# xkuubix/MonteCarlo-Gated-MIL

Measured on AMD Instinct MI355X. Metric: bags/sec × MCDO-samples (T=100) at N=2048,d=512; 1/2/4/8-GPU + %HBM roofline, higher is better.
Workload: dtype bf16

## Files before the change

montecarlo-gated-mil_amd/csrc/mcgmil_kernels.h:

```cpp
#pragma once
#include "mcgmil_device.h"

namespace mcgmil {

struct GateParams {
    const void* H;
    long long ldh;
    const int32_t* bag_off;
    int B, T, L, D, C, G, P;
    long long total_samples;
    const void* Wp;
    uint32_t wp_bytes;
    const float* bv;
    const float* bu;
    const float* wa;
    const float* ba;
    float sf, sa;
    uint32_t thr_f, thr_a;
    uint32_t thrx_f;
    uint32_t k0, k1;
    uint32_t bag_base;
    int t_base;
    const uint32_t* bag_ids;
    const int32_t* tile_bag;
// ... 3 lines not shown
    float* logits;
    float* zz;
    float* Y;
    float* A;
    const int32_t* region_off;
    int region_t;
    unsigned long long* stamps;
    unsigned long long* clock;
    long long tile_row0;
};

constexpr int kClockSlots = 1024;
__device__ __forceinline__ void clock_probe(const GateParams& p, int i) {
    if (p.clock && threadIdx.x == 0 && blockIdx.x < (unsigned)kClockSlots) {
        const unsigned long long t = __builtin_amdgcn_s_memtime();
        const unsigned long long r = __builtin_amdgcn_s_memrealtime();
        p.clock[(size_t)blockIdx.x * 4 + 2 * i] = t;
        p.clock[(size_t)blockIdx.x * 4 + 2 * i + 1] = r;
    }
}

#ifdef MCGMIL_STAMPS
#define MCGMIL_STAMP(p, i)                                                                 \
    do {                                                                                    \
        __builtin_amdgcn_sched_barrier(0);                                                  \
        if (threadIdx.x == 0 && (p).stamps)                                                 \
            (p).stamps[(size_t)blockIdx.x * 8 + (i)] = __builtin_amdgcn_s_memtime();        \
        __builtin_amdgcn_sched_barrier(0);                                                  \
    } while (0)
#else
#define MCGMIL_STAMP(p, i) do {} while (0)
#endif


constexpr int kGateThreads = 512;
constexpr int kGateWaves = kGateThreads / kWave;
constexpr int kRowInfo = 6;


template <int BM, int RV = BM>
__device__ __forceinline__ void fill_row_table(const GateParams& p, long long R0, int* rinfo) {
    const int tid = threadIdx.x;
    if (tid >= BM) return;
    const long long R = tid < RV ? R0 + tid : p.total_samples;
    int hrow = -1, t = 0, n = 0, bag = 0, Nb = 0;
    const bool narrow = p.total_samples <= 0xFFFFFFFFll;
    if (R < p.total_samples && p.uniform_rows > 0) {
        const long long per_bag = (long long)p.T * p.uniform_rows;
        Nb = p.uniform_rows;
        if (narrow) {
            const uint32_t r = (uint32_t)R, pb = (uint32_t)per_bag;
            bag = (int)(r / pb);
            const uint32_t local = r - (uint32_t)bag * pb;
            t = (int)(local / (uint32_t)Nb);
            n = (int)(local - (uint32_t)t * (uint32_t)Nb);
        } else {
            bag = (int)(R / per_bag);
            const long long local = R - (long long)bag * per_bag;
            t = (int)(local / Nb);
            n = (int)(local - (long long)t * Nb);
        }
        hrow = bag * Nb + n;
    } else if (R < p.total_samples) {
        if (p.tile_bag) {
            bag = p.tile_bag[R0 / BM];
            while ((long long)p.T * p.bag_off[bag + 1] <= R) ++bag;
        } else {
            bag = find_bag(p.bag_off, p.B, p.T, R);
        }
        const int ob = p.bag_off[bag];
        Nb = p.bag_off[bag + 1] - ob;
        const long long local = R - (long long)p.T * ob;
        if (narrow) {
            t = (int)((uint32_t)local / (uint32_t)Nb);
            n = (int)((uint32_t)local - (uint32_t)t * (uint32_t)Nb);
        } else {
            t = (int)(local / Nb);
            n = (int)(local - (long long)t * Nb);
        }
        hrow = ob + n;
    }
    int* ri = rinfo + kRowInfo * tid;
    ri[0] = hrow; ri[1] = t; ri[2] = n; ri[3] = bag; ri[4] = Nb;
    ri[5] = (int)(p.bag_ids ? p.bag_ids[bag] : p.bag_base + (uint32_t)bag);
}

#ifndef MCGMIL_KERNELS_TEMPLATES_ONLY
__global__ void plan_tiles_kernel(const int32_t* bag_off, int B, int T, long long total_samples,
                                  int BM, long long tiles, int32_t* tile_bag) {
    const long long i = (long long)blockIdx.x * blockDim.x + threadIdx.x;
    if (i >= tiles) return;
    const long long R = i * BM;
    tile_bag[i] = R < total_samples ? find_bag(bag_off, B, T, R) : 0;
}
#endif

__device__ __forceinline__ float gated_product_scaled(float ax, float by) {
    ax = fminf(fmaxf(ax, -43.280851226668903f), 43.280851226668903f);
    const float a = __builtin_amdgcn_exp2f(ax);
    const float b = __builtin_amdgcn_exp2f(by);
    const float ia = 1.0f + a;
    return (1.0f - a) * __builtin_amdgcn_rcpf(fmaf(ia, b, ia));
}

#ifndef MCGMIL_DIAG
#define MCGMIL_DIAG 0
#endif
#ifndef MCGMIL_PHILOX_ROUNDS
#define MCGMIL_PHILOX_ROUNDS 10
#endif

constexpr float kM2Log2e = -2.8853900817779268f;
constexpr float kMLog2e = -1.4426950408889634f;

struct HeadVec { f32x4 bv, bu, wa; };

template <int PPW>
__device__ __forceinline__ void load_head_vectors(const GateParams& p, int q0, int lane,
                                                  HeadVec (&hv)[PPW]) {
    const int DB = p.D >> 4;
#pragma unroll
    for (int jp = 0; jp < PPW; ++jp) {
        const int q = q0 + jp < p.P ? q0 + jp : p.P - 1;
        const int g = q / DB, db = q - g * DB;
        const int d0 = db * 16 + 4 * (lane >> 4);
        hv[jp].bv = *reinterpret_cast<const f32x4*>(p.bv + (size_t)g * p.D + d0) * kM2Log2e;
        hv[jp].bu = *reinterpret_cast<const f32x4*>(p.bu + (size_t)g * p.D + d0) * kMLog2e;
        hv[jp].wa = *reinterpret_cast<const f32x4*>(p.wa + (size_t)g * p.D + d0);
    }
}

struct Region {
    int bag, t0, t1, Nb, ob;
    int ntiles;
    long long S, rows;
};

constexpr int kFusedTiles = 32;
constexpr int kFusedHv = 256;
struct alignas(16) FusedConst {
    Region rg;
    uint32_t bagctr;
    int pad0;
    float ba[4];
    int cls[8];
    int pad1[8];
    int4 tile[kFusedTiles];
    float hv[3][kFusedHv];
};

#ifndef MCGMIL_FUSED_HV_LDS
#define MCGMIL_FUSED_HV_LDS 1
#endif
template <int PPW>
__device__ __forceinline__ void load_head_vectors_lds(const FusedConst* fc, int P, int q0, int lane,
                                                      HeadVec (&hv)[PPW]) {
#pragma unroll
    for (int jp = 0; jp < PPW; ++jp) {
        const int q = q0 + jp < P ? q0 + jp : P - 1;
        const int d = 16 * q + 4 * (lane >> 4);
        hv[jp].bv = *reinterpret_cast<const f32x4*>(fc->hv[0] + d);
        hv[jp].bu = *reinterpret_cast<const f32x4*>(fc->hv[1] + d);
        hv[jp].wa = *reinterpret_cast<const f32x4*>(fc->hv[2] + d);
    }
}

template <int RT, int PPW, int MAXC, bool ONE_CLASS, int RTV = RT>
__device__ __forceinline__ void fold_pairs(const GateParams& p, const f32x4 (&acc)[RT][2 * PPW],
                                           int q0, int lane, float (&part)[MAXC][RT],
                                           const HeadVec* pre = nullptr) {
    const int DB = p.D >> 4;
    const float av_s = p.sf * kM2Log2e, au_s = p.sf * kMLog2e;
#pragma unroll
    for (int jp = 0; jp < PPW; ++jp) {
        const int q = q0 + jp;
        if (q >= p.P) break;
        const int col = 16 * q + 4 * (lane >> 4);
        const int g = ONE_CLASS ? 0 : q / DB;
        const int d0 = col - g * p.D;
        f32x4 bvv, buv;
        f32x4 coef[MAXC];
        if (ONE_CLASS && pre) {
            bvv = pre[jp].bv;
            buv = pre[jp].bu;
            coef[0] = pre[jp].wa;
#pragma unroll
            for (int c = 1; c < MAXC; ++c) coef[c] = f32x4{0.f, 0.f, 0.f, 0.f};
        } else {
            bvv = *reinterpret_cast<const f32x4*>(p.bv + col);
            buv = *reinterpret_cast<const f32x4*>(p.bu + col);
            bvv *= kM2Log2e;
            buv *= kMLog2e;
#pragma unroll
            for (int c = 0; c < MAXC; ++c) {
                const int cc = ONE_CLASS ? g : c;
                const bool use = ONE_CLASS ? (c == 0) : ((c < p.C) && (p.G == 1 || c == g));
                const f32x4 w = *reinterpret_cast<const f32x4*>(p.wa + (size_t)(use ? cc : 0) * p.D + d0);
                coef[c] = use ? w : f32x4{0.f, 0.f, 0.f, 0.f};
            }
        }
#pragma unroll
        for (int rt = 0; rt < RTV; ++rt) {
#pragma unroll
            for (int v = 0; v < 4; ++v) {
                const float ax = fmaf(acc[rt][2 * jp][v], av_s, bvv[v]);
                const float by = fmaf(acc[rt][2 * jp + 1][v], au_s, buv[v]);
                if constexpr (ONE_CLASS) {
#if MCGMIL_DIAG & 8
                    part[0][rt] = fmaf(fmaf(ax, coef[0][v], by), ax, part[0][rt]);
                    continue;
#endif
                    const float a = __builtin_amdgcn_exp2f(fminf(fmaxf(ax, -43.280851226668903f),
                                                                 43.280851226668903f));
                    const float b = __builtin_amdgcn_exp2f(by);
                    const float ia = 1.0f + a;
                    const float r = __builtin_amdgcn_rcpf(fmaf(ia, b, ia));
                    part[0][rt] = fmaf(fmaf(-a, coef[0][v], coef[0][v]), r, part[0][rt]);
                } else {
                    const float pr = gated_product_scaled(ax, by);
#pragma unroll
                    for (int c = 0; c < MAXC; ++c) part[c][rt] = fmaf(pr, coef[c][v], part[c][rt]);
                }
            }
        }
    }
}

template <int BM, int MAXC>
__host__ __device__ constexpr int red_floats() { return kGateWaves * MAXC * 4 * BM; }

template <int BM, int MAXC, int ROWS = 16, bool AFFINE = false>
__device__ __forceinline__ void finish_scores(const GateParams& p, long long R0,
                                              float (&part)[MAXC][BM / ROWS], f32x4 zacc,
                                              bool zwave, float* red, float* zred,
                                              const int* rinfo, int one_class, int waves_per_gate,
                                              bool have_keep, bool keep, float* lg_out,
                                              float* z_out, long long obase,
                                              const FusedConst* fc = nullptr, int tile = 0) {
    constexpr int RT = BM / ROWS;
    constexpr int NG = 64 / ROWS;
    const int tid = threadIdx.x, lane = tid & 63, wave = tid >> 6;
    const int ncls = one_class < 0 ? MAXC : 1;
#pragma unroll
    for (int c = 0; c < MAXC; ++c) {
        if (c >= ncls) break;
        const int cls = one_class < 0 ? c : one_class;
        if (cls >= MAXC) break;
        float* dst = red + ((size_t)(wave * MAXC + cls) * NG + lane / ROWS) * BM + (lane % ROWS);
#pragma unroll
        for (int q = 0; q < RT; ++q) dst[ROWS * q] = part[c][q];
    }
    if (zwave && lane < 16) {
#pragma unroll
        for (int c = 0; c < MAXC; ++c) zred[c * BM + wave * 16 + lane] = zacc[c];
    }
    MCGMIL_STAMP(p, 5);
    __syncthreads();
    MCGMIL_STAMP(p, 6);
    const int r = wave * 16 + (lane & 15), c = lane >> 4;
    if (r >= BM || c >= p.C) return;
    int t, n, bag, Nb;
    uint32_t bagc;
    size_t orow;
    float bias;
    if constexpr (AFFINE) {
        const int4 tl = fc->tile[tile];
        t = tl.x, n = tl.y + r, bag = fc->rg.bag, Nb = fc->rg.Nb;
        bagc = fc->bagctr;
        orow = (size_t)(tl.z + r);
        bias = fc->ba[c];
    } else {
        const int* ri = rinfo + kRowInfo * r;
        if (ri[0] < 0) return;
        t = ri[1], n = ri[2], bag = ri[3], Nb = ri[4];
        bagc = (uint32_t)ri[5];
        orow = (size_t)(R0 + r - obase);
        bias = p.ba[c];
    }
    float s = 0.f;
    const int nw = waves_per_gate ? waves_per_gate : kGateWaves;
    for (int k = 0; k < nw; ++k) {
        const int w = waves_per_gate ? c * waves_per_gate + k : k;
        const float* src = red + (size_t)(w * MAXC + c) * NG * BM + r;
#pragma unroll
        for (int g = 0; g < NG; ++g) s += src[g * BM];
    }
    s += bias;
    if (p.keep_att) {
        const size_t abase = (size_t)p.T * p.C * (size_t)p.bag_off[bag];
        keep = p.keep_att[abase + ((size_t)t * p.C + c) * Nb + n] != 0;
    } else if (!have_keep) {
        keep = attention_keep(p.k0, p.k1, bagc, (uint32_t)(p.t_base + t), (uint32_t)c,
                              (uint32_t)n, p.thr_a);
    }
    const size_t o = orow * p.C + c;
    lg_out[o] = s * (keep ? p.sa : 0.f);
    z_out[o] = zred[c * BM + r] * p.sf;
}

constexpr int kSoftmaxRows = 16;

#ifndef MCGMIL_NT_A
#define MCGMIL_NT_A 1
#endif
__device__ __forceinline__ void store_a(float* dst, float v) {
#if MCGMIL_NT_A
    __builtin_nontemporal_store(v, dst);
#else
    *dst = v;
#endif
}

__device__ __forceinline__ void softmax_group(int ltid, bool active, int Nb, int C, const float* lg,
                                              const float* zz, float* Ao, float* Yo, float* sred) {
    const int tid = ltid, lane = ltid & 63, wave = ltid >> 6;
    if (Nb == 0) {
        if (active && tid < C) Yo[tid] = 0.f;
        return;
    }
    const int Nl = active ? Nb : 0;
    if (C == 2 && Nb <= 256 * kSoftmaxRows) {
        float (*sred2)[4] = reinterpret_cast<float (*)[4]>(sred);
        float e0[kSoftmaxRows], e1[kSoftmaxRows];
        float2 zr[kSoftmaxRows];
        float m0 = -INFINITY, m1 = -INFINITY;
#pragma unroll
        for (int k = 0; k < kSoftmaxRows; ++k) {
            const int n = tid + 256 * k;
            float2 l = make_float2(-INFINITY, -INFINITY);
            zr[k] = make_float2(0.f, 0.f);
            if (n < Nl) {
                l = *reinterpret_cast<const float2*>(lg + (size_t)n * 2);
                zr[k] = *reinterpret_cast<const float2*>(zz + (size_t)n * 2);
            }
            e0[k] = l.x;
            e1[k] = l.y;
            m0 = fmaxf(m0, e0[k]);
            m1 = fmaxf(m1, e1[k]);
        }
        m0 = wave_max(m0);
        m1 = wave_max(m1);
        if (lane == 0) { sred2[0][wave] = m0; sred2[1][wave] = m1; }
        __syncthreads();
        m0 = fmaxf(fmaxf(sred2[0][0], sred2[0][1]), fmaxf(sred2[0][2], sred2[0][3]));
        m1 = fmaxf(fmaxf(sred2[1][0], sred2[1][1]), fmaxf(sred2[1][2], sred2[1][3]));
        __syncthreads();
        float s0 = 0.f, y0 = 0.f, s1 = 0.f, y1 = 0.f;
#pragma unroll
        for (int k = 0; k < kSoftmaxRows; ++k) {
            const int n = tid + 256 * k;
            if (n < Nl) {
                const float2 z = zr[k];
                e0[k] = expf(e0[k] - m0);
                e1[k] = expf(e1[k] - m1);
                s0 += e0[k];
                s1 += e1[k];
                y0 = fmaf(e0[k], z.x, y0);
                y1 = fmaf(e1[k], z.y, y1);
            }
        }
        s0 = wave_sum(s0);
        y0 = wave_sum(y0);
        s1 = wave_sum(s1);
        y1 = wave_sum(y1);
        if (lane == 0) {
            sred2[0][wave] = s0; sred2[1][wave] = y0; sred2[2][wave] = s1; sred2[3][wave] = y1;
        }
        __syncthreads();
        s0 = (sred2[0][0] + sred2[0][1]) + (sred2[0][2] + sred2[0][3]);
        y0 = (sred2[1][0] + sred2[1][1]) + (sred2[1][2] + sred2[1][3]);
        s1 = (sred2[2][0] + sred2[2][1]) + (sred2[2][2] + sred2[2][3]);
        y1 = (sred2[3][0] + sred2[3][1]) + (sred2[3][2] + sred2[3][3]);
        __syncthreads();
        const float inv0 = 1.0f / s0, inv1 = 1.0f / s1;
        if (Ao) {
            float* Ao1 = Ao + Nb;
#pragma unroll
            for (int k = 0; k < kSoftmaxRows; ++k) {
                const int n = tid + 256 * k;
                if (n < Nl) {
                    store_a(Ao + n, e0[k] * inv0);
                    store_a(Ao1 + n, e1[k] * inv1);
                }
            }
        }
        if (active && tid == 0) { Yo[0] = y0 * inv0; Yo[1] = y1 * inv1; }
        return;
    }
    float (*sr)[4] = reinterpret_cast<float (*)[4]>(sred);
    for (int c = 0; c < C; ++c) {
        if (Nb <= 256 * kSoftmaxRows) {
            float e[kSoftmaxRows];
            float m = -INFINITY;
#pragma unroll
            for (int k = 0; k < kSoftmaxRows; ++k) {
                const int n = tid + 256 * k;
                e[k] = n < Nl ? lg[(size_t)n * C + c] : -INFINITY;
                m = fmaxf(m, e[k]);
            }
            m = wave_max(m);
            if (lane == 0) sr[0][wave] = m;
            __syncthreads();
            m = fmaxf(fmaxf(sr[0][0], sr[0][1]), fmaxf(sr[0][2], sr[0][3]));
            __syncthreads();
            float s = 0.f, y = 0.f;
#pragma unroll
            for (int k = 0; k < kSoftmaxRows; ++k) {
                const int n = tid + 256 * k;
                if (n < Nl) {
                    e[k] = expf(e[k] - m);
                    s += e[k];
                    y = fmaf(e[k], zz[(size_t)n * C + c], y);
                }
            }
            s = wave_sum(s);
            y = wave_sum(y);
            if (lane == 0) { sr[0][wave] = s; sr[1][wave] = y; }
            __syncthreads();
            s = (sr[0][0] + sr[0][1]) + (sr[0][2] + sr[0][3]);
            y = (sr[1][0] + sr[1][1]) + (sr[1][2] + sr[1][3]);
            __syncthreads();
            const float inv = 1.0f / s;
            if (Ao) {
                float* Aoc = Ao + (size_t)c * Nb;
#pragma unroll
                for (int k = 0; k < kSoftmaxRows; ++k) {
                    const int n = tid + 256 * k;
                    if (n < Nl) store_a(Aoc + n, e[k] * inv);
                }
            }
            if (active && tid == 0) Yo[c] = y * inv;
            continue;
        }
        float m = -INFINITY;
        for (int n = tid; n < Nl; n += 256) m = fmaxf(m, lg[(size_t)n * C + c]);
        m = wave_max(m);
        if (lane == 0) sr[0][wave] = m;
        __syncthreads();
        m = fmaxf(fmaxf(sr[0][0], sr[0][1]), fmaxf(sr[0][2], sr[0][3]));
        __syncthreads();
        float s = 0.f, y = 0.f;
        for (int n = tid; n < Nl; n += 256) {
            const size_t o = (size_t)n * C + c;
            const float e = expf(lg[o] - m);
            s += e;
            y = fmaf(e, zz[o], y);
        }
        s = wave_sum(s);
        y = wave_sum(y);
        if (lane == 0) { sr[0][wave] = s; sr[1][wave] = y; }
        __syncthreads();
        s = (sr[0][0] + sr[0][1]) + (sr[0][2] + sr[0][3]);
        y = (sr[1][0] + sr[1][1]) + (sr[1][2] + sr[1][3]);
        __syncthreads();
        const float inv = 1.0f / s;
        if (Ao) {
            float* Aoc = Ao + (size_t)c * Nb;
            for (int n = tid; n < Nl; n += 256) store_a(Aoc + n, expf(lg[(size_t)n * C + c] - m) * inv);
        }
        if (active && tid == 0) Yo[c] = y * inv;
    }
}

#ifndef MCGMIL_KERNELS_TEMPLATES_ONLY
__global__ __launch_bounds__(256) void softmax_pool_kernel(const int32_t* bag_off, int T, int C,
                                                           const float* logits, const float* zz,
                                                           float* Y, float* A) {
    __shared__ float sred[16];
    const int t = blockIdx.x, b = blockIdx.y;
    const int ob = bag_off[b];
    const int Nb = bag_off[b + 1] - ob;
    const size_t R0 = (size_t)T * ob + (size_t)t * Nb;
    softmax_group(threadIdx.x, true, Nb, C, logits + R0 * C, zz + R0 * C,
                  A ? A + (size_t)T * C * ob + (size_t)t * C * Nb : nullptr,
                  Y + ((size_t)b * T + t) * C, sred);
}
#endif

template <typename E> struct Raw;
template <> struct Raw<__bf16> { uint4 v; };
template <> struct Raw<float> { f32x4 lo, hi; };
__device__ __forceinline__ Raw<__bf16> load_raw(const __bf16* p) {
    Raw<__bf16> r; r.v = *reinterpret_cast<const uint4*>(p); return r;
}
__device__ __forceinline__ Raw<float> load_raw(const float* p) {
    Raw<float> r;
    r.lo = *reinterpret_cast<const f32x4*>(p);
    r.hi = *reinterpret_cast<const f32x4*>(p + 4);
    return r;
}
__device__ __forceinline__ void store_masked(const Raw<__bf16>& h, uint32_t kb, __bf16* dst) {
    uint4 v = h.v;
    v.x &= ((kb & 1u) ? 0x0000FFFFu : 0u) | ((kb & 2u) ? 0xFFFF0000u : 0u);
    v.y &= ((kb & 4u) ? 0x0000FFFFu : 0u) | ((kb & 8u) ? 0xFFFF0000u : 0u);
    v.z &= ((kb & 16u) ? 0x0000FFFFu : 0u) | ((kb & 32u) ? 0xFFFF0000u : 0u);
    v.w &= ((kb & 64u) ? 0x0000FFFFu : 0u) | ((kb & 128u) ? 0xFFFF0000u : 0u);
    *reinterpret_cast<uint4*>(dst) = v;
}
__device__ __forceinline__ void store_masked(const Raw<float>& h, uint32_t kb, float* dst) {
    f32x4 a = h.lo, b = h.hi;
    a.x = (kb & 1u) ? a.x : 0.f;   a.y = (kb & 2u) ? a.y : 0.f;
    a.z = (kb & 4u) ? a.z : 0.f;   a.w = (kb & 8u) ? a.w : 0.f;
    b.x = (kb & 16u) ? b.x : 0.f;  b.y = (kb & 32u) ? b.y : 0.f;
    b.z = (kb & 64u) ? b.z : 0.f;  b.w = (kb & 128u) ? b.w : 0.f;
    *reinterpret_cast<f32x4*>(dst) = a;
    *reinterpret_cast<f32x4*>(dst + 4) = b;
}

__device__ __forceinline__ void store_dropped(const Raw<__bf16>& h, uint4 o, uint32_t thrx,
                                              uint32_t inval, __bf16* dst) {
    uint4 v = h.v;
    v.x = __builtin_amdgcn_bitop3_b32(v.x, drop_mask16x2_flipped(o.x, thrx), inval, 0x10);
    v.y = __builtin_amdgcn_bitop3_b32(v.y, drop_mask16x2(o.y, thrx), inval, 0x10);
    v.z = __builtin_amdgcn_bitop3_b32(v.z, drop_mask16x2_flipped(o.z, thrx), inval, 0x10);
    v.w = __builtin_amdgcn_bitop3_b32(v.w, drop_mask16x2(o.w, thrx), inval, 0x10);
    *reinterpret_cast<uint4*>(dst) = v;
}
__device__ __forceinline__ uint32_t keep_lo(uint32_t m) { return ~(uint32_t)((int32_t)(m << 16) >> 16); }
__device__ __forceinline__ uint32_t keep_hi(uint32_t m) { return ~(uint32_t)((int32_t)m >> 16); }
__device__ __forceinline__ void store_dropped(const Raw<float>& h, uint4 o, uint32_t thrx,
                                              uint32_t inval, float* dst) {
    const uint32_t m0 = drop_mask16x2_flipped(o.x, thrx) | inval, m1 = drop_mask16x2(o.y, thrx) | inval;
    const uint32_t m2 = drop_mask16x2_flipped(o.z, thrx) | inval, m3 = drop_mask16x2(o.w, thrx) | inval;
    f32x4 a = h.lo, b = h.hi;
    a.x = __uint_as_float(__float_as_uint(a.x) & keep_lo(m0));
    a.y = __uint_as_float(__float_as_uint(a.y) & keep_hi(m0));
    a.z = __uint_as_float(__float_as_uint(a.z) & keep_lo(m1));
    a.w = __uint_as_float(__float_as_uint(a.w) & keep_hi(m1));
    b.x = __uint_as_float(__float_as_uint(b.x) & keep_lo(m2));
    b.y = __uint_as_float(__float_as_uint(b.y) & keep_hi(m2));
    b.z = __uint_as_float(__float_as_uint(b.z) & keep_lo(m3));
    b.w = __uint_as_float(__float_as_uint(b.w) & keep_hi(m3));
    *reinterpret_cast<f32x4*>(dst) = a;
    *reinterpret_cast<f32x4*>(dst + 4) = b;
}

constexpr int kPipeBM = 128;
#ifndef MCGMIL_VPM
#define MCGMIL_VPM 2
#endif
constexpr int VPM = MCGMIL_VPM;
#ifndef MCGMIL_SCHED
#define MCGMIL_SCHED 0
#endif
constexpr int HD = 2;
template <typename E>
__host__ __device__ constexpr int pipe_slots() { return 2; }

template <typename E, int MAXC>
__host__ __device__ constexpr size_t pipe_lds_bytes() {
    return (size_t)pipe_slots<E>() * kPipeBM * 32 * sizeof(E) + (size_t)red_floats<kPipeBM, MAXC>() * 4 +
           (size_t)MAXC * kPipeBM * 4 + (size_t)kRowInfo * kPipeBM * 4;
}

template <typename E>
__device__ __forceinline__ void load_classifier_lds(__amdgpu_buffer_rsrc_t wrs, uint32_t zsoff, int KS, E* zw) {
    for (int i = threadIdx.x; i < KS * 64; i += kGateThreads)
        *reinterpret_cast<f32x4*>(zw + (size_t)i * 8) = __builtin_bit_cast(
            f32x4, __builtin_amdgcn_raw_buffer_load_b128(wrs, (uint32_t)i * 8u * (uint32_t)sizeof(E), zsoff, 0));
}

template <typename E, int PPW, int MAXC, bool REPLAY, bool ONE_CLASS, bool EARLY_HV = true,
          bool ZL = false, bool ZLOAD = true, int RTV = kPipeBM / 16, bool AFFINE = false>
__device__ __forceinline__ void pipe_tile(const GateParams& p, long long R0, E* Xs, float* red,
                                          float* zred, const int* rinfo, float* lg_out,
                                          float* z_out, long long obase, E* zw = nullptr,
                                          const FusedConst* fc = nullptr, int tile = 0) {
    constexpr int BM = kPipeBM;
    constexpr int RT = BM / 16;
    constexpr int NJ = 2 * PPW;
    constexpr int SLOT = RT * 64 * 8;
    const int tid = threadIdx.x, lane = tid & 63, wave = tid >> 6;
    const int KS = p.L >> 5;

    int hrow;
    uint32_t cn, ct, cb;
    if constexpr (AFFINE) {
        static_assert(!REPLAY, "the affine rows have no replay masks");
        const int4 tl = fc->tile[tile];
        cn = (uint32_t)(tl.y + wave * 16 + (lane & 15));
        hrow = fc->rg.ob + (int)cn;
        ct = (uint32_t)(p.t_base + tl.x);
        cb = fc->bagctr;
    } else {
        const int* ri = rinfo + kRowInfo * (wave * 16 + (lane & 15));
        hrow = ri[0];
        cn = (uint32_t)ri[2], ct = (uint32_t)(p.t_base + ri[1]), cb = (uint32_t)ri[5];
    }
    const bool valid = AFFINE || hrow >= 0;
    const int kq = lane >> 4;
    const E* hsrc = reinterpret_cast<const E*>(p.H) + (size_t)(valid ? hrow : 0) * p.ldh + kq * 8;
    const uint8_t* kfe = REPLAY ? p.keep_feat + (size_t)(valid ? R0 + wave * 16 + (lane & 15) : 0) *
                                                    (p.L >> 3) + kq
                                : nullptr;

    const uint32_t inval = valid ? 0u : 0xFFFFFFFFu;
    auto stage = [&](int s, const Raw<E>& h, E* slot) {
        if constexpr (REPLAY) {
            const uint32_t kb = kfe[(size_t)(s < KS ? s : KS - 1) * 4];
            store_masked(h, kb & ~inval, slot + tid * 8);
        } else {
#if MCGMIL_DIAG & 4
            const uint4 o = make_uint4(cn * 0x9E3779B9u + (uint32_t)s, ct ^ cb, cn + ct, (uint32_t)s * 77u);
#else
            const uint4 o = philox4x32_10<true, MCGMIL_PHILOX_ROUNDS>((uint32_t)(s * 4 + kq), cn, ct, cb, p.k0, p.k1);
#endif
            store_dropped(h, o, p.thrx_f, inval, slot + tid * 8);
        }
    };

    const __amdgpu_buffer_rsrc_t wrs = make_rsrc(p.Wp, p.wp_bytes);
    const uint32_t tile_bytes = (uint32_t)KS * 512u * (uint32_t)sizeof(E);
    constexpr uint32_t kStepBytes = 512u * (uint32_t)sizeof(E);
    const int q0 = __builtin_amdgcn_readfirstlane(wave) * PPW;
    uint32_t wsoff[NJ];
#pragma unroll
    for (int j = 0; j < NJ; ++j) {
        int q = q0 + (j >> 1);
        q = q < p.P ? q : p.P - 1;
        wsoff[j] = (uint32_t)(2 * q + (j & 1)) * tile_bytes;
    }
    const uint32_t zsoff = (uint32_t)(2 * p.P) * tile_bytes;
    const uint32_t lane_b = (uint32_t)lane * 8u * (uint32_t)sizeof(E);
    auto wfrag = [&](uint32_t soff) { return load_frag_buf<E>(wrs, lane_b, soff); };

    f32x4 acc[RT][NJ];
#pragma unroll
    for (int rt = 0; rt < RT; ++rt)
#pragma unroll
        for (int j = 0; j < NJ; ++j) acc[rt][j] = f32x4{0.f, 0.f, 0.f, 0.f};
    f32x4 zacc = {0.f, 0.f, 0.f, 0.f};

    auto kstep = [&](int s, const E* cur, E* nxt, const Frag<E> (&w)[NJ], const Frag<E>& z,
                     Frag<E> (&wn)[NJ], Frag<E>& zn, const Raw<E>& h, Raw<E>& hn) {
        const int s1 = s + 1 < KS ? s + 1 : KS - 1;
        const int sh = s + HD < KS ? s + HD : KS - 1;
#if MCGMIL_DIAG & 2
#pragma unroll
        for (int j = 0; j < NJ; ++j) wn[j] = w[j];
        zn = z;
#else
#pragma unroll
        for (int j = 0; j < NJ; ++j) wn[j] = wfrag(wsoff[j] + (uint32_t)s1 * kStepBytes);
        if constexpr (!ZL) zn = wfrag(zsoff + (uint32_t)s1 * kStepBytes);
#endif
#if MCGMIL_DIAG & 1
        hn = h;
#else
        if (RTV == RT || wave < RTV) hn = load_raw(hsrc + (size_t)sh * 32);
#endif
#pragma unroll
        for (int rt = 0; rt < RTV; ++rt) {
            const Frag<E> x = load_frag(cur + (size_t)(rt * 64 + lane) * 8);
#pragma unroll
            for (int j = 0; j < NJ; ++j) acc[rt][j] = mma(w[j], x, acc[rt][j]);
        }
        const Frag<E> xz = load_frag(cur + (size_t)tid * 8);
        if constexpr (ZL) zacc = mma(load_frag(zw + (size_t)(s * 64 + lane) * 8), xz, zacc);
        else zacc = mma(z, xz, zacc);
        if (RTV == RT || wave < RTV) stage(s + 1, h, nxt);
        if constexpr (sizeof(E) == 2 && PPW == 2) {
#if MCGMIL_SCHED == 1
            __builtin_amdgcn_sched_group_barrier(0x020, NJ + 2, 0);
            __builtin_amdgcn_sched_group_barrier(0x100, 3, 0);
#pragma unroll
            for (int rt = 0; rt < RT; ++rt) {
#pragma unroll
                for (int j = 0; j < NJ; ++j) {
                    __builtin_amdgcn_sched_group_barrier(0x008, 1, 0);
                    __builtin_amdgcn_sched_group_barrier(0x002, VPM, 0);
                }
                if (rt + 2 < RT) __builtin_amdgcn_sched_group_barrier(0x100, 1, 0);
            }
            __builtin_amdgcn_sched_group_barrier(0x008, 1, 0);
            __builtin_amdgcn_sched_group_barrier(0x002, VPM, 0);
#else
#pragma unroll
            for (int i = 0; i < RTV * NJ + 1; ++i) {
                __builtin_amdgcn_sched_group_barrier(0x008, 1, 0);
                __builtin_amdgcn_sched_group_barrier(0x002, VPM, 0);
            }
#endif
        }
#if MCGMIL_DIAG & 128
        asm volatile("s_waitcnt lgkmcnt(0)" ::: "memory");
#else
        __syncthreads();
#endif
    };

    constexpr bool kEarlyHV = EARLY_HV && ONE_CLASS && sizeof(E) == 2;
    HeadVec hvec[PPW];
    {
        Frag<E> wA[NJ], wB[NJ], zA, zB;
        Raw<E> hA{}, hB{};
        if (RTV == RT || wave < RTV) {
            hA = load_raw(hsrc);
            hB = load_raw(hsrc + 32);
        }
#pragma unroll
        for (int j = 0; j < NJ; ++j) wA[j] = wfrag(wsoff[j]);
        if constexpr (ZL) {
            if constexpr (ZLOAD) load_classifier_lds<E>(wrs, zsoff, KS, zw);
        } else {
            zA = wfrag(zsoff);
        }
        if (RTV == RT || wave < RTV) stage(0, hA, Xs);
        __syncthreads();
        MCGMIL_STAMP(p, 2);

        if constexpr (kEarlyHV) load_head_vectors<PPW>(p, q0, lane, hvec);
        kstep(0, Xs, Xs + SLOT, wA, zA, wB, zB, hB, hA);
        kstep(1, Xs + SLOT, Xs, wB, zB, wA, zA, hA, hB);
#if MCGMIL_DIAG & 16
        if (KS > 1000)
#endif
        for (int s = 2; s < KS; s += 2) {
            kstep(s, Xs, Xs + SLOT, wA, zA, wB, zB, hB, hA);
            kstep(s + 1, Xs + SLOT, Xs, wB, zB, wA, zA, hA, hB);
        }
    }
    MCGMIL_STAMP(p, 3);

    float part[MAXC][RT];
#pragma unroll
    for (int c = 0; c < MAXC; ++c)
#pragma unroll
        for (int rt = 0; rt < RT; ++rt) part[c][rt] = 0.f;
    constexpr bool kLdsHV = MCGMIL_FUSED_HV_LDS && AFFINE && ONE_CLASS && !kEarlyHV;
    if constexpr (kLdsHV) load_head_vectors_lds<PPW>(fc, p.P, q0, lane, hvec);
    fold_pairs<RT, PPW, MAXC, ONE_CLASS, RTV>(p, acc, q0, lane, part, kEarlyHV || kLdsHV ? hvec : nullptr);
    MCGMIL_STAMP(p, 4);
    int one_class = -1;
    if constexpr (ONE_CLASS && AFFINE) one_class = __builtin_amdgcn_readfirstlane(fc->cls[wave]);
    else if constexpr (ONE_CLASS) one_class = q0 < p.P ? q0 / (p.D >> 4) : MAXC;
    finish_scores<BM, MAXC, 16, AFFINE>(p, R0, part, zacc, true, red, zred, rinfo, one_class,
                                        ONE_CLASS ? (p.D >> 4) / PPW : 0, false, true, lg_out, z_out,
                                        obase, fc, tile);
    MCGMIL_STAMP(p, 7);
}

#ifndef MCGMIL_XCD_TILES
#define MCGMIL_XCD_TILES 1
#endif
__device__ __forceinline__ long long xcd_tile(unsigned b, unsigned n, int bags) {
#if MCGMIL_XCD_TILES
    const unsigned x = b & 7u, q = n >> 3, r = n & 7u;
    const unsigned l = (x < r ? x * (q + 1) : r * (q + 1) + (x - r) * q) + (b >> 3);
    return (long long)(bags >= 8 ? l : b);
#else
    (void)n;
    (void)bags;
    return (long long)b;
#endif
}

template <typename E, int PPW, int MAXC, bool REPLAY, bool ONE_CLASS, bool PROBE = false, int RTV = kPipeBM / 16>
__global__ __launch_bounds__(kGateThreads) void gate_pipe_kernel(const GateParams p) {
    extern __shared__ __attribute__((aligned(16))) unsigned char smem[];
    constexpr int BM = kPipeBM;
    E* Xs = reinterpret_cast<E*>(smem);
    float* red = reinterpret_cast<float*>(smem + (size_t)pipe_slots<E>() * BM * 32 * sizeof(E));
    float* zred = red + red_floats<BM, MAXC>();
    int* rinfo = reinterpret_cast<int*>(zred + MAXC * BM);
    const long long R0 = RTV == BM / 16 ? xcd_tile(blockIdx.x, gridDim.x, p.B) * BM
                                        : p.tile_row0 + (long long)blockIdx.x * (16 * RTV);

    if constexpr (PROBE) clock_probe(p, 0);
    MCGMIL_STAMP(p, 0);
    fill_row_table<BM, 16 * RTV>(p, R0, rinfo);
    __syncthreads();
    MCGMIL_STAMP(p, 1);
    pipe_tile<E, PPW, MAXC, REPLAY, ONE_CLASS, true, false, true, RTV>(p, R0, Xs, red, zred, rinfo, p.logits,
                                                                       p.zz, 0);
    if constexpr (PROBE) clock_probe(p, 1);
}

#ifndef MCGMIL_FUSED_XCD
#define MCGMIL_FUSED_XCD 1
#endif
#ifndef MCGMIL_FUSED_EARLY_HV
#define MCGMIL_FUSED_EARLY_HV 0
#endif
#ifndef MCGMIL_FUSED_NMAJOR
#define MCGMIL_FUSED_NMAJOR 1
#endif
#ifndef MCGMIL_FUSED_CAP
#define MCGMIL_FUSED_CAP 4096
#endif
template <int MAXC>
__host__ __device__ constexpr int fused_cap() { return MAXC <= 2 ? MCGMIL_FUSED_CAP : MCGMIL_FUSED_CAP / 4; }

template <typename E, int MAXC>
__host__ __device__ constexpr size_t fused_lds_bytes() {
    return pipe_lds_bytes<E, MAXC>() + (size_t)kRowInfo * kPipeBM * 4
           + (size_t)2 * fused_cap<MAXC>() * MAXC * 4
           + (size_t)2 * 16 * 4 + sizeof(FusedConst);
}
static_assert(kFusedTiles * kPipeBM >= MCGMIL_FUSED_CAP, "FusedConst::tile holds a whole region");

__host__ __device__ inline bool fused_affine(int uniform_rows, int cap) {
    return uniform_rows > 0 && uniform_rows % kPipeBM == 0 && uniform_rows <= cap;
}

#ifndef MCGMIL_FUSED_ZL
#define MCGMIL_FUSED_ZL 1
#endif
template <typename E>
__host__ __device__ constexpr bool fused_zl() { return MCGMIL_FUSED_ZL && sizeof(E) == 2; }
template <typename E, int MAXC>
__host__ __device__ constexpr size_t fused_kernel_lds_bytes(int L) {
    return fused_lds_bytes<E, MAXC>() + (fused_zl<E>() ? (size_t)(L / 32) * 512 * sizeof(E) : 0);
}

__host__ __device__ inline int region_t_groups(int Nb, int T, int cap) {
    if (Nb <= 0) return T;
    if (Nb > cap) return 1;
    const int ts = cap / Nb;
    return ts < T ? ts : T;
}

__device__ __forceinline__ int region_tile(const Region& rg, int i) {
#if MCGMIL_FUSED_NMAJOR
    const int G = rg.t1 - rg.t0;
    if (G > 1 && rg.Nb % kPipeBM == 0) return (i % G) * (rg.Nb / kPipeBM) + i / G;
#endif
    return i;
}

__device__ __forceinline__ GateParams reload_kernarg_params(const GateParams& p) {
#if __HIP_DEVICE_COMPILE__
    typedef __attribute__((address_space(4))) const GateParams* KernargParams;
    KernargParams q = (KernargParams)__builtin_amdgcn_kernarg_segment_ptr();
    asm volatile("" : "+s"(q));
    return *q;
#else
    return p;
#endif
}

__device__ __forceinline__ bool decode_region(const GateParams& p, int g, int cap, Region& rg) {
    int b, j, ts;
    if (p.uniform_rows > 0) {
        ts = p.region_t;
        const int rpb = (p.T + ts - 1) / ts;
        if (MCGMIL_FUSED_XCD && (p.B & 7) == 0) {
            const int k = g >> 3;
            b = 8 * (k / rpb) + (g & 7);
            j = k - (k / rpb) * rpb;
        } else {
            b = g / rpb;
            j = g - b * rpb;
        }
        if (b >= p.B) return false;
    } else {
        if (g >= p.region_off[p.B]) return false;
        b = find_bag(p.region_off, p.B, 1, g);
        j = g - p.region_off[b];
        ts = region_t_groups(p.bag_off[b + 1] - p.bag_off[b], p.T, cap);
    }
    rg.bag = b;
    rg.ob = p.bag_off[b];
    rg.Nb = p.bag_off[b + 1] - rg.ob;
    rg.t0 = j * ts;
    rg.t1 = rg.t0 + ts < p.T ? rg.t0 + ts : p.T;
    rg.S = (long long)p.T * rg.ob + (long long)rg.t0 * rg.Nb;
    rg.rows = (long long)(rg.t1 - rg.t0) * rg.Nb;
    rg.ntiles = (int)((rg.rows + kPipeBM - 1) / kPipeBM);
    return true;
}

template <int BM>
__device__ __forceinline__ void fill_row_table_region(const GateParams& p, const Region& rg,
                                                      long long R0, int* rinfo) {
    const int tid = threadIdx.x;
    if (tid >= BM) return;
    const long long rho = R0 + tid - rg.S;
    int hrow = -1, t = 0, n = 0;
    if (rho < rg.rows) {
        const uint32_t r = (uint32_t)rho;
        const uint32_t tt = r / (uint32_t)rg.Nb;
        n = (int)(r - tt * (uint32_t)rg.Nb);
        t = rg.t0 + (int)tt;
        hrow = rg.ob + n;
    }
    int* ri = rinfo + kRowInfo * tid;
    ri[0] = hrow; ri[1] = t; ri[2] = n; ri[3] = rg.bag; ri[4] = rg.Nb;
    ri[5] = (int)(p.bag_ids ? p.bag_ids[rg.bag] : p.bag_base + (uint32_t)rg.bag);
}


template <int PPW, int MAXC, bool ONE_CLASS>
__device__ __forceinline__ void fill_fused_const(const GateParams& p, const Region& rg, FusedConst* fc) {
    const int tid = threadIdx.x;
    if (tid == 0) {
        fc->rg = rg;
        fc->bagctr = p.bag_ids ? p.bag_ids[rg.bag] : p.bag_base + (uint32_t)rg.bag;
    }
    if (tid < MAXC) fc->ba[tid] = tid < p.C ? p.ba[tid] : 0.f;
    if (tid < kGateWaves) {
        const int q0 = tid * PPW, DB = p.D >> 4;
        int g = 0;
        while ((g + 1) * DB <= q0) ++g;
        fc->cls[tid] = ONE_CLASS && q0 < p.P ? g : MAXC;
    }
    if (tid < rg.ntiles && tid < kFusedTiles) {
        const int G = rg.t1 - rg.t0, nbt = rg.Nb / kPipeBM;
        const int dv = MCGMIL_FUSED_NMAJOR ? G : nbt;
        int qt = 0;
        while ((qt + 1) * dv <= tid) ++qt;
        const int rem = tid - qt * dv;
        const int tg = MCGMIL_FUSED_NMAJOR ? rem : qt, nb = MCGMIL_FUSED_NMAJOR ? qt : rem;
        fc->tile[tid] = make_int4(rg.t0 + tg, nb * kPipeBM, tg * rg.Nb + nb * kPipeBM, 0);
    }
    if (ONE_CLASS && tid < 16 * p.P && tid < kFusedHv) {
        fc->hv[0][tid] = p.bv[tid] * kM2Log2e;
        fc->hv[1][tid] = p.bu[tid] * kMLog2e;
        fc->hv[2][tid] = p.wa[tid];
    }
}

template <typename E, int PPW, int MAXC, bool ONE_CLASS, bool PROBE, bool AFFINE>
__device__ __forceinline__ void fused_region(const GateParams& p) {
    extern __shared__ __attribute__((aligned(16))) unsigned char smem[];
    constexpr int BM = kPipeBM;
    constexpr int CAP = fused_cap<MAXC>();
    E* Xs = reinterpret_cast<E*>(smem);
    float* red = reinterpret_cast<float*>(smem + (size_t)pipe_slots<E>() * BM * 32 * sizeof(E));
    float* zred = red + red_floats<BM, MAXC>();
    int* rinfo = reinterpret_cast<int*>(zred + MAXC * BM);
    float* slg = reinterpret_cast<float*>(rinfo + 2 * kRowInfo * BM);
    float* szz = slg + CAP * MAXC;
    float* sred = szz + CAP * MAXC;
    FusedConst* fc = reinterpret_cast<FusedConst*>(sred + 32);

#if MCGMIL_DIAG & 64
    {
        const long long R0 = (long long)blockIdx.x * BM;
        fill_row_table<BM>(p, R0, rinfo);
        __syncthreads();
        pipe_tile<E, PPW, MAXC, false, ONE_CLASS>(p, R0, Xs, red, zred, rinfo, p.logits, p.zz, 0);
        return;
    }
#endif
    Region rg;
    if (!decode_region(p, (int)blockIdx.x, CAP, rg)) return;
    if constexpr (PROBE) clock_probe(p, 0);
    const int ntiles = (int)((rg.rows + BM - 1) / BM);
    Region* srg = &fc->rg;
    if constexpr (AFFINE) fill_fused_const<PPW, MAXC, ONE_CLASS>(p, rg, fc);
    else if (threadIdx.x == 0) *srg = rg;
    __syncthreads();
    E* zw = reinterpret_cast<E*>(smem + fused_lds_bytes<E, MAXC>());
    if constexpr (fused_zl<E>())
        load_classifier_lds<E>(make_rsrc(p.Wp, p.wp_bytes), (uint32_t)(2 * p.P) * (uint32_t)(p.L >> 5) * 512u *
                                   (uint32_t)sizeof(E), p.L >> 5, zw);
    for (int i = 0; i < ntiles; ++i) {
        const GateParams pt = reload_kernarg_params(p);
        if constexpr (AFFINE) {
            MCGMIL_STAMP(pt, 0);
            MCGMIL_STAMP(pt, 1);
            pipe_tile<E, PPW, MAXC, false, ONE_CLASS, MCGMIL_FUSED_EARLY_HV, fused_zl<E>(), false, BM / 16, true>(
                pt, 0, Xs, red, zred, nullptr, slg, szz, 0, zw, fc, i);
        } else {
            Region* qr = srg;
            asm volatile("" : "+v"(qr));
            int* ri = rinfo + (i & 1) * kRowInfo * BM;
            MCGMIL_STAMP(pt, 0);
            {
                const Region r = *qr;
                fill_row_table_region<BM>(pt, r, r.S + (long long)region_tile(r, i) * BM, ri);
            }
            __syncthreads();
            MCGMIL_STAMP(pt, 1);
            const Region r = *qr;
            const bool lds = r.Nb <= CAP;
            pipe_tile<E, PPW, MAXC, false, ONE_CLASS, MCGMIL_FUSED_EARLY_HV, fused_zl<E>(), false>(
                pt, r.S + (long long)region_tile(r, i) * BM, Xs, red, zred, ri, lds ? slg : pt.logits,
                lds ? szz : pt.zz, lds ? r.S : 0, zw);
        }
    }
    __syncthreads();
#if MCGMIL_DIAG & 32
    if (ntiles >= 0) return;
#endif
    rg = *srg;
    const bool in_lds = AFFINE || rg.Nb <= CAP;

    const int G = rg.t1 - rg.t0;
    const int half = threadIdx.x >> 8, ltid = threadIdx.x & 255;
    for (int j0 = 0; j0 < G; j0 += 2) {
        const bool act = j0 + half < G;
        const int j = act ? j0 + half : j0;
        const long long row0 = (long long)j * rg.Nb;
        const float* lgj = in_lds ? slg + row0 * p.C : p.logits + (rg.S + row0) * p.C;
        const float* zzj = in_lds ? szz + row0 * p.C : p.zz + (rg.S + row0) * p.C;
        float* Ao = p.A ? p.A + (size_t)p.T * p.C * rg.ob + (size_t)(rg.t0 + j) * p.C * rg.Nb : nullptr;
        float* Yo = p.Y + ((size_t)rg.bag * p.T + rg.t0 + j) * p.C;
        softmax_group(ltid, act, rg.Nb, p.C, lgj, zzj, Ao, Yo, sred + half * 16);
    }
    if constexpr (PROBE) clock_probe(p, 1);
}

template <typename E, int PPW, int MAXC, bool ONE_CLASS, bool PROBE = false>
__global__ __launch_bounds__(kGateThreads) void gate_fused_kernel(const GateParams p) {
    fused_region<E, PPW, MAXC, ONE_CLASS, PROBE, true>(p);
}

template <typename E, int PPW, int MAXC, bool ONE_CLASS, bool PROBE = false>
__global__ __launch_bounds__(kGateThreads) void gate_fused_table_kernel(const GateParams p) {
    fused_region<E, PPW, MAXC, ONE_CLASS, PROBE, false>(p);
}

template <int BM>
__host__ __device__ constexpr int gate_row_info_ints() { return kRowInfo * BM; }

template <typename E, int BM, int MAXC>
__host__ __device__ constexpr size_t gate_lds_bytes(int L) {
    const size_t tile = (size_t)BM * L * sizeof(E), red = (size_t)red_floats<BM, MAXC>() * 4;
    return (tile > red ? tile : red) + (size_t)MAXC * BM * 4 + (size_t)gate_row_info_ints<BM>() * 4;
}

template <typename E, int BM, int PPW, int MAXC>
__global__ __launch_bounds__(kGateThreads) void gate_scores_kernel(const GateParams p) {
    extern __shared__ __attribute__((aligned(16))) unsigned char smem[];
    constexpr int RT = BM / 16;
    constexpr int NJ = 2 * PPW;
    const int tid = threadIdx.x;
    const int lane = tid & 63;
    const int wave = tid >> 6;
    const int L = p.L;
    const int KS = L >> 5;
    const int LC = L >> 3;

    E* Xs = reinterpret_cast<E*>(smem);
    float* red = reinterpret_cast<float*>(smem);
    const size_t tile_bytes = (size_t)BM * L * sizeof(E), red_bytes = (size_t)red_floats<BM, MAXC>() * 4;
    float* zred = reinterpret_cast<float*>(smem + (tile_bytes > red_bytes ? tile_bytes : red_bytes));
    int* rinfo = reinterpret_cast<int*>(zred + MAXC * BM);
    const long long R0 = (long long)blockIdx.x * BM;

    fill_row_table<BM>(p, R0, rinfo);
    __syncthreads();

    {
        const E* H = reinterpret_cast<const E*>(p.H);
        const int items = BM * LC;
        for (int i = tid; i < items; i += kGateThreads) {
            const int blk = i >> 6, slot = i & 63;
            const int rt = blk / KS, ks = blk - rt * KS;
            const int r = rt * 16 + (slot & 15);
            const int kc = ks * 4 + (slot >> 4);
            E* dst = Xs + ((size_t)blk * 64 + slot) * 8;
            const int* ri = rinfo + kRowInfo * r;
            const int hrow = ri[0];
            if (hrow < 0) {
                store_zero8(dst);
                continue;
            }
            uint32_t kb;
            if (p.keep_feat) {
                kb = p.keep_feat[(size_t)(R0 + r) * LC + kc];
            } else {
                const uint4 o = philox4x32_10((uint32_t)kc, (uint32_t)ri[2],
                                              (uint32_t)(p.t_base + ri[1]), (uint32_t)ri[5],
                                              p.k0, p.k1);
                kb = keep_byte(o, p.thr_f);
            }
            load_masked(H + (size_t)hrow * p.ldh + (size_t)kc * 8, kb, dst);
        }
    }
    __syncthreads();

    const E* Wp = reinterpret_cast<const E*>(p.Wp);
    const int pairs_per_pass = kGateWaves * PPW;
    const int npass = (p.P + pairs_per_pass - 1) / pairs_per_pass;
    const size_t tile_elems = (size_t)KS * 512;

    float part[MAXC][RT];
#pragma unroll
    for (int c = 0; c < MAXC; ++c)
#pragma unroll
        for (int rt = 0; rt < RT; ++rt) part[c][rt] = 0.f;
    f32x4 zacc = {0.f, 0.f, 0.f, 0.f};
    const bool zwave = wave < RT;

    for (int pass = 0; pass < npass; ++pass) {
        const int q0 = pass * pairs_per_pass + wave * PPW;
        const bool active = q0 < p.P;
        const bool doz = (pass == 0) && zwave;
        if (!active && !doz) continue;

        f32x4 acc[RT][NJ];
#pragma unroll
        for (int rt = 0; rt < RT; ++rt)
#pragma unroll
            for (int j = 0; j < NJ; ++j) acc[rt][j] = f32x4{0.f, 0.f, 0.f, 0.f};

        const E* wbase[NJ];
#pragma unroll
        for (int j = 0; j < NJ; ++j) {
            int q = q0 + (j >> 1);
            q = q < p.P ? q : p.P - 1;
            wbase[j] = Wp + (size_t)(2 * q + (j & 1)) * tile_elems + lane * 8;
        }
        const E* zbase = Wp + (size_t)(2 * p.P) * tile_elems + lane * 8;

        Frag<E> wcur[NJ], wnxt[NJ];
        Frag<E> zcur = zero_frag<E>(), znxt = zero_frag<E>();
#pragma unroll
        for (int j = 0; j < NJ; ++j) wcur[j] = active ? load_frag(wbase[j]) : zero_frag<E>();
        if (doz) zcur = load_frag(zbase);

        for (int ks = 0; ks < KS; ++ks) {
            if (ks + 1 < KS) {
#pragma unroll
// ... 174 lines not shown
```

Before: 985,200.

## Chain tile prologues across fused tiles and precompute attention keep bits in LDS

```diff
diff --git a/montecarlo-gated-mil_amd/csrc/mcgmil_kernels.h b/montecarlo-gated-mil_amd/csrc/mcgmil_kernels.h
--- a/montecarlo-gated-mil_amd/csrc/mcgmil_kernels.h
+++ b/montecarlo-gated-mil_amd/csrc/mcgmil_kernels.h
@@ -179,6 +179,13 @@
 #ifndef MCGMIL_FUSED_HV_LDS
 #define MCGMIL_FUSED_HV_LDS 1
 #endif
+#ifndef MCGMIL_FUSED_ATT_LDS
+#define MCGMIL_FUSED_ATT_LDS 1
+#endif
+#ifndef MCGMIL_FUSED_CHAIN
+#define MCGMIL_FUSED_CHAIN 1
+#endif
+
 template <int PPW>
 __device__ __forceinline__ void load_head_vectors_lds(const FusedConst* fc, int P, int q0, int lane,
                                                       HeadVec (&hv)[PPW]) {
@@ -263,7 +270,8 @@
                                               const int* rinfo, int one_class, int waves_per_gate,
                                               bool have_keep, bool keep, float* lg_out,
                                               float* z_out, long long obase,
-                                              const FusedConst* fc = nullptr, int tile = 0) {
+                                              const FusedConst* fc = nullptr, int tile = 0,
+                                              const uint8_t* att = nullptr) {
     constexpr int RT = BM / ROWS;
     constexpr int NG = 64 / ROWS;
     const int tid = threadIdx.x, lane = tid & 63, wave = tid >> 6;
@@ -284,15 +292,22 @@
     MCGMIL_STAMP(p, 5);
     __syncthreads();
     MCGMIL_STAMP(p, 6);
-    const int r = wave * 16 + (lane & 15), c = lane >> 4;
+    int r = wave * 16 + (lane & 15), c = lane >> 4;
+    if constexpr (AFFINE) {
+        int ts = tid;
+        asm volatile("" : "+v"(ts));
+        r = (ts >> 6) * 16 + (ts & 15), c = (ts >> 4) & 3;
+    }
     if (r >= BM || c >= p.C) return;
     int t, n, bag, Nb;
     uint32_t bagc;
     size_t orow;
     float bias;
+    int akb = 0;
     if constexpr (AFFINE) {
         const int4 tl = fc->tile[tile];
         t = tl.x, n = tl.y + r, bag = fc->rg.bag, Nb = fc->rg.Nb;
+        akb = tl.w + c * (Nb >> 3) + (r >> 3);
         bagc = fc->bagctr;
         orow = (size_t)(tl.z + r);
         bias = fc->ba[c];
@@ -316,6 +331,8 @@
     if (p.keep_att) {
         const size_t abase = (size_t)p.T * p.C * (size_t)p.bag_off[bag];
         keep = p.keep_att[abase + ((size_t)t * p.C + c) * Nb + n] != 0;
+    } else if (AFFINE && MCGMIL_FUSED_ATT_LDS) {
+        keep = (att[akb] >> (r & 7)) & 1;
     } else if (!have_keep) {
         keep = attention_keep(p.k0, p.k1, bagc, (uint32_t)(p.t_base + t), (uint32_t)c,
                               (uint32_t)n, p.thr_a);
@@ -587,12 +604,19 @@
             f32x4, __builtin_amdgcn_raw_buffer_load_b128(wrs, (uint32_t)i * 8u * (uint32_t)sizeof(E), zsoff, 0));
 }
 
+template <int M> struct StepMode { static constexpr int value = M; };
+template <typename E, int NJ> struct TileCarry {
+    Frag<E> w[NJ];
+    Raw<E> h;
+};
 template <typename E, int PPW, int MAXC, bool REPLAY, bool ONE_CLASS, bool EARLY_HV = true,
           bool ZL = false, bool ZLOAD = true, int RTV = kPipeBM / 16, bool AFFINE = false>
 __device__ __forceinline__ void pipe_tile(const GateParams& p, long long R0, E* Xs, float* red,
                                           float* zred, const int* rinfo, float* lg_out,
                                           float* z_out, long long obase, E* zw = nullptr,
-                                          const FusedConst* fc = nullptr, int tile = 0) {
+                                          const FusedConst* fc = nullptr, int tile = 0,
+                                          int next_tile = 0, TileCarry<E, 2 * PPW>* carry = nullptr,
+                                          const uint8_t* att = nullptr) {
     constexpr int BM = kPipeBM;
     constexpr int RT = BM / 16;
     constexpr int NJ = 2 * PPW;
@@ -622,7 +646,7 @@
                                 : nullptr;
 
     const uint32_t inval = valid ? 0u : 0xFFFFFFFFu;
-    auto stage = [&](int s, const Raw<E>& h, E* slot) {
+    auto stage = [&](int s, const Raw<E>& h, E* slot, uint32_t cn, uint32_t ct, int kq) {
         if constexpr (REPLAY) {
             const uint32_t kb = kfe[(size_t)(s < KS ? s : KS - 1) * 4];
             store_masked(h, kb & ~inval, slot + tid * 8);
@@ -658,9 +682,14 @@
         for (int j = 0; j < NJ; ++j) acc[rt][j] = f32x4{0.f, 0.f, 0.f, 0.f};
     f32x4 zacc = {0.f, 0.f, 0.f, 0.f};
 
-    auto kstep = [&](int s, const E* cur, E* nxt, const Frag<E> (&w)[NJ], const Frag<E>& z,
+    constexpr bool kChain = MCGMIL_FUSED_CHAIN && AFFINE && ZL && !ZLOAD && sizeof(E) == 2 && RTV == RT;
+    const E* hnext = hsrc;
+    uint32_t cnn = cn, ctn = ct;
+    int kqn = kq;
+    auto kstep = [&](auto mode, int s, const E* cur, E* nxt, const Frag<E> (&w)[NJ], const Frag<E>& z,
                      Frag<E> (&wn)[NJ], Frag<E>& zn, const Raw<E>& h, Raw<E>& hn) {
-        const int s1 = s + 1 < KS ? s + 1 : KS - 1;
+        constexpr int M = decltype(mode)::value;
+        const int s1 = M == 2 ? 0 : s + 1 < KS ? s + 1 : KS - 1;
         const int sh = s + HD < KS ? s + HD : KS - 1;
 #if MCGMIL_DIAG & 2
 #pragma unroll
@@ -674,7 +703,8 @@
 #if MCGMIL_DIAG & 1
         hn = h;
 #else
-        if (RTV == RT || wave < RTV) hn = load_raw(hsrc + (size_t)sh * 32);
+        if constexpr (M != 0) hn = load_raw(hnext + (M - 1) * 32);
+        else if (RTV == RT || wave < RTV) hn = load_raw(hsrc + (size_t)sh * 32);
 #endif
 #pragma unroll
         for (int rt = 0; rt < RTV; ++rt) {
@@ -685,7 +715,8 @@
         const Frag<E> xz = load_frag(cur + (size_t)tid * 8);
         if constexpr (ZL) zacc = mma(load_frag(zw + (size_t)(s * 64 + lane) * 8), xz, zacc);
         else zacc = mma(z, xz, zacc);
-        if (RTV == RT || wave < RTV) stage(s + 1, h, nxt);
+        if constexpr (M == 2) stage(0, h, nxt, cnn, ctn, kqn);
+        else if (RTV == RT || wave < RTV) stage(s + 1, h, nxt, cn, ct, kq);
         if constexpr (sizeof(E) == 2 && PPW == 2) {
 #if MCGMIL_SCHED == 1
             __builtin_amdgcn_sched_group_barrier(0x020, NJ + 2, 0);
@@ -721,30 +752,57 @@
     {
         Frag<E> wA[NJ], wB[NJ], zA, zB;
         Raw<E> hA{}, hB{};
-        if (RTV == RT || wave < RTV) {
-            hA = load_raw(hsrc);
-            hB = load_raw(hsrc + 32);
-        }
-#pragma unroll
-        for (int j = 0; j < NJ; ++j) wA[j] = wfrag(wsoff[j]);
-        if constexpr (ZL) {
-            if constexpr (ZLOAD) load_classifier_lds<E>(wrs, zsoff, KS, zw);
+        const bool chained = kChain && KS > 2 && tile > 0;
+        if (chained) {
+            if constexpr (kChain) {
+#pragma unroll
+                for (int j = 0; j < NJ; ++j) wA[j] = carry->w[j];
+                hB = carry->h;
+            }
         } else {
-            zA = wfrag(zsoff);
-        }
-        if (RTV == RT || wave < RTV) stage(0, hA, Xs);
-        __syncthreads();
+            if (RTV == RT || wave < RTV) {
+                hA = load_raw(hsrc);
+                hB = load_raw(hsrc + 32);
+            }
+#pragma unroll
+            for (int j = 0; j < NJ; ++j) wA[j] = wfrag(wsoff[j]);
+            if constexpr (ZL) {
+                if constexpr (ZLOAD) load_classifier_lds<E>(wrs, zsoff, KS, zw);
+            } else {
+                zA = wfrag(zsoff);
+            }
+            if (RTV == RT || wave < RTV) stage(0, hA, Xs, cn, ct, kq);
+            __syncthreads();
+        }
         MCGMIL_STAMP(p, 2);
 
         if constexpr (kEarlyHV) load_head_vectors<PPW>(p, q0, lane, hvec);
-        kstep(0, Xs, Xs + SLOT, wA, zA, wB, zB, hB, hA);
-        kstep(1, Xs + SLOT, Xs, wB, zB, wA, zA, hA, hB);
+        constexpr StepMode<0> body{};
+        kstep(body, 0, Xs, Xs + SLOT, wA, zA, wB, zB, hB, hA);
+        kstep(body, 1, Xs + SLOT, Xs, wB, zB, wA, zA, hA, hB);
+        const int kend = kChain && KS > 2 ? KS - 2 : KS;
 #if MCGMIL_DIAG & 16
         if (KS > 1000)
 #endif
-        for (int s = 2; s < KS; s += 2) {
-            kstep(s, Xs, Xs + SLOT, wA, zA, wB, zB, hB, hA);
-            kstep(s + 1, Xs + SLOT, Xs, wB, zB, wA, zA, hA, hB);
+        for (int s = 2; s < kend; s += 2) {
+            kstep(body, s, Xs, Xs + SLOT, wA, zA, wB, zB, hB, hA);
+            kstep(body, s + 1, Xs + SLOT, Xs, wB, zB, wA, zA, hA, hB);
+        }
+        if constexpr (kChain) {
+            if (KS > 2) {
+                int tq = tid;
+                asm volatile("" : "+v"(tq));
+                const int4 tn = fc->tile[next_tile];
+                kqn = (tq >> 4) & 3;
+                cnn = (uint32_t)(tn.y + (tq >> 6) * 16 + (tq & 15));
+                ctn = (uint32_t)(p.t_base + tn.x);
+                hnext = reinterpret_cast<const E*>(p.H) + (size_t)(fc->rg.ob + (int)cnn) * p.ldh + kqn * 8;
+                kstep(StepMode<1>{}, KS - 2, Xs, Xs + SLOT, wA, zA, wB, zB, hB, hA);
+                kstep(StepMode<2>{}, KS - 1, Xs + SLOT, Xs, wB, zB, wA, zA, hA, hB);
+            }
+#pragma unroll
+            for (int j = 0; j < NJ; ++j) carry->w[j] = wA[j];
+            carry->h = hB;
         }
     }
     MCGMIL_STAMP(p, 3);
@@ -763,7 +821,7 @@
     else if constexpr (ONE_CLASS) one_class = q0 < p.P ? q0 / (p.D >> 4) : MAXC;
     finish_scores<BM, MAXC, 16, AFFINE>(p, R0, part, zacc, true, red, zred, rinfo, one_class,
                                         ONE_CLASS ? (p.D >> 4) / PPW : 0, false, true, lg_out, z_out,
-                                        obase, fc, tile);
+                                        obase, fc, tile, att);
     MCGMIL_STAMP(p, 7);
 }
 
@@ -938,12 +996,30 @@
         while ((qt + 1) * dv <= tid) ++qt;
         const int rem = tid - qt * dv;
         const int tg = MCGMIL_FUSED_NMAJOR ? rem : qt, nb = MCGMIL_FUSED_NMAJOR ? qt : rem;
-        fc->tile[tid] = make_int4(rg.t0 + tg, nb * kPipeBM, tg * rg.Nb + nb * kPipeBM, 0);
+        fc->tile[tid] = make_int4(rg.t0 + tg, nb * kPipeBM, tg * rg.Nb + nb * kPipeBM,
+                                  tg * p.C * (rg.Nb >> 3) + nb * (kPipeBM >> 3));
     }
     if (ONE_CLASS && tid < 16 * p.P && tid < kFusedHv) {
         fc->hv[0][tid] = p.bv[tid] * kM2Log2e;
         fc->hv[1][tid] = p.bu[tid] * kMLog2e;
         fc->hv[2][tid] = p.wa[tid];
+    }
+}
+
+template <int MAXC>
+__device__ __forceinline__ void fill_att_keep(const GateParams& p, const Region& rg, uint8_t* att) {
+    static_assert((size_t)fused_cap<MAXC>() * MAXC / 8 <= (size_t)2 * kRowInfo * kPipeBM * 4,
+                  "the region's keep bytes fit the row tables' LDS");
+    const uint32_t nb8 = (uint32_t)rg.Nb >> 3, per = (uint32_t)p.C * nb8;
+    const uint32_t total = (uint32_t)(rg.t1 - rg.t0) * per;
+    const uint32_t bagc = p.bag_ids ? p.bag_ids[rg.bag] : p.bag_base + (uint32_t)rg.bag;
+    const float rper = __builtin_amdgcn_rcpf((float)per), rnb8 = __builtin_amdgcn_rcpf((float)nb8);
+    for (uint32_t i = threadIdx.x; i < total; i += kGateThreads) {
+        const uint32_t tg = (uint32_t)(((float)i + 0.5f) * rper), rem = i - tg * per;
+        const uint32_t c = (uint32_t)(((float)rem + 0.5f) * rnb8), nb = rem - c * nb8;
+        const uint4 o = philox4x32_10(nb, c, (uint32_t)(p.t_base + rg.t0 + (int)tg) | 0x80000000u, bagc,
+                                      p.k0, p.k1);
+        att[i] = (uint8_t)keep_byte(o, p.thr_a);
     }
 }
 
@@ -982,13 +1058,18 @@
     if constexpr (fused_zl<E>())
         load_classifier_lds<E>(make_rsrc(p.Wp, p.wp_bytes), (uint32_t)(2 * p.P) * (uint32_t)(p.L >> 5) * 512u *
                                    (uint32_t)sizeof(E), p.L >> 5, zw);
+    uint8_t* att = reinterpret_cast<uint8_t*>(rinfo);
+    if constexpr (AFFINE && MCGMIL_FUSED_ATT_LDS) {
+        if (!p.keep_att) fill_att_keep<MAXC>(p, rg, att);
+    }
+    [[maybe_unused]] TileCarry<E, 2 * PPW> carry;
     for (int i = 0; i < ntiles; ++i) {
         const GateParams pt = reload_kernarg_params(p);
         if constexpr (AFFINE) {
             MCGMIL_STAMP(pt, 0);
             MCGMIL_STAMP(pt, 1);
             pipe_tile<E, PPW, MAXC, false, ONE_CLASS, MCGMIL_FUSED_EARLY_HV, fused_zl<E>(), false, BM / 16, true>(
-                pt, 0, Xs, red, zred, nullptr, slg, szz, 0, zw, fc, i);
+                pt, 0, Xs, red, zred, nullptr, slg, szz, 0, zw, fc, i, i + 1 < ntiles ? i + 1 : i, &carry, att);
         } else {
             Region* qr = srg;
             asm volatile("" : "+v"(qr));
```

Result: no change. 994,100, median of 6 (+0.9%).
